# liuQuan98/EYOC

Measured on AMD Instinct MI355X. Metric: registered pairs/sec (30k-voxel KITTI pairs), higher is better.
Workload: dtype f32 (split16 products: fp32 storage/accumulation, 3 fp16 MFMAs on hi/lo-split operands per product); 1 GPU; 64 synthetic 30 cm KITTI-shaped pairs per step per GPU (mean 29894 voxels/cloud, ResUNetBN2C random-init, 5000-point NN, RANSAC 4000000 hypotheses/pair, planted inlier ratio 0.3, spconv math split16); parallelism=pairs sharded over 1 GPU(s), steps_in_flight=2

## Files before the change

eyoc_amd/_lib.py:

```python
from __future__ import annotations

import ctypes as C
import os
import threading

_HERE = os.path.dirname(os.path.abspath(__file__))
LIB_PATH = os.environ.get("EYOC_HIP_LIB") or os.path.join(_HERE, "lib", "libeyoc_hip.so")

MAX_LEVELS = 4
MAP_S1, MAP_DOWN, MAP_UP = 0, 1, 2


class MapsInfo(C.Structure):
    _fields_ = [("n_levels", C.c_int32), ("rows", C.c_int32 * MAX_LEVELS),
                ("pairs_s1", C.c_int64 * MAX_LEVELS), ("pairs_down", C.c_int64 * MAX_LEVELS),
                ("pairs_up", C.c_int64 * MAX_LEVELS), ("pairs_conv1", C.c_int64)]


class ModelDesc(C.Structure):
    _fields_ = [("in_channels", C.c_int32), ("out_channels", C.c_int32), ("conv1_kernel_size", C.c_int32),
                ("normalize_feature", C.c_int32), ("channels", C.c_int32 * 5), ("tr_channels", C.c_int32 * 5),
                ("bn_eps", C.c_float), ("expanded", C.c_int32)]


# ... 101 lines not shown
    "eyoc_spconv_grad_weight": (_i, [_vp, _vp, _i, _i, _vp, _i, _i, _vp, _i, _i, _vp, _vp, _sz, _vp]),
    "eyoc_spconv_pack_weights_split16": (_i, [_vp, _vp, _i, _i, _i, _vp, _vp]),
    "eyoc_spconv_ex": (_i, [_vp, _vp, _i, _i, _i, _vp, _i, _i, _vp, _i, _vp, _vp, _i, _i, _vp, _i, _i, _i, _vp, _vp]),
    "eyoc_spconv_select_split16_kernel": (_i, [_vp, _i]),
    "eyoc_spconv_select_st_kernel": (_i, [_vp, _i]),
    "eyoc_spconv_st_split_below": (_i, [_vp, _i]),
    "eyoc_spconv_st_group_rows": (_i, [_vp, _i]),
    "eyoc_spconv_st_ksplit": (_i, [_vp, _i]),
    "eyoc_spconv_local_rulebook_bytes": (_sz, [_i]),
    "eyoc_spconv_build_local_rulebook": (_i, [_vp, _vp, _i, _i, _vp, _vp, _vp]),
    "eyoc_spconv_staged": (_i, [_vp, _vp, _vp, _i, _i, _vp, _i, _i, _vp, _i, _vp, _vp, _i, _i, _vp, _i, _i, _vp, _vp]),
    "eyoc_split16_encode": (_i, [_vp, _vp, _i, _i, _i, _vp, _i, _vp]),
    "eyoc_split16_decode": (_i, [_vp, _vp, _i, _i, _i, _vp, _i, _vp]),
    "eyoc_model_set_math": (_i, [_vp, _i]),
    "eyoc_model_last_math": (_i, [_vp]),
    "eyoc_model_range_check": (_i, [_vp, _vp, C.POINTER(C.c_float)]),
    "eyoc_model_range_snapshot": (_i, [_vp, _vp, _vp]),
    "eyoc_model_set_progress_event": (_i, [_vp, _i, _vp]),
    "eyoc_model_set_probe": (_i, [_vp, _i]),
    "eyoc_spconv": (_i, [_vp, _vp, _i, _i, _vp, _i, _i, _vp, _i, _vp, _vp, _i, _i, _vp, _i, _vp]),
    "eyoc_spconv_sum": (_i, [_vp, _vp, _i, _i, _vp, _i, _i, _vp, _i, _vp, _i, _vp]),
    "eyoc_model_blob_floats": (_sz, [C.POINTER(ModelDesc)]),
    "eyoc_model_pack_host": (_i, [C.POINTER(ModelDesc), C.POINTER(LayerParams), _i, _vp, _sz]),
    "eyoc_model_create": (_i, [_vp, C.POINTER(ModelDesc), C.POINTER(LayerParams), _i, _vp, _sz, C.POINTER(_vp)]),
    "eyoc_model_destroy": (_i, [_vp]),
    "eyoc_model_repack_workspace_bytes": (_sz, [_vp]),
    "eyoc_model_repack_device": (_i, [_vp, _vp, C.POINTER(LayerParams), _i, _vp, _sz, _vp]),
    "eyoc_model_fuse_tail": (_i, [_vp, _i]),
    "eyoc_model_workspace_bytes": (_sz, [_vp, _vp]),
    "eyoc_model_forward": (_i, [_vp, _vp, _vp, _vp, _vp, _vp, _sz, _vp]),
    "eyoc_model_workspace_bytes_rows": (_sz, [_vp, _vp, _i]),
    "eyoc_model_forward_rows": (_i, [_vp, _vp, _vp, _vp, _vp, _i, _vp, _vp, _sz, _vp]),
    "eyoc_model_sampled_tail": (_i, [_vp, _i]),
    "eyoc_model_num_layers": (_i, [_vp]),
    "eyoc_model_layer_work": (_i, [_vp, _vp, _vp, _vp, C.POINTER(C.c_char_p), C.POINTER(C.c_int64),
                                   C.POINTER(C.c_double), C.POINTER(C.c_double), C.POINTER(C.c_double)]),
    "eyoc_model_set_timing": (_i, [_vp, _i]),
    "eyoc_model_layer_ms": (_i, [_vp, C.POINTER(C.c_float)]),
    "eyoc_model_timing_slot": (_i, [_vp, _i]),
    "eyoc_bn_workspace_bytes": (_sz, [_i, _i]),
    "eyoc_bn_train_forward": (_i, [_vp, _vp, _i, _i, _i, _vp, _vp, C.c_float, _i, _vp, _i, _vp, _vp, _sz, _vp]),
    "eyoc_bn_train_forward_running": (_i, [_vp, _vp, _i, _i, _i, _vp, _vp, C.c_float, _i, _vp, _i, _vp, _vp, _vp, C.c_float, _vp, _sz, _vp]),
    "eyoc_bn_train_backward": (_i, [_vp, _vp, _i, _vp, _i, _vp, _i, _i, _i, _vp, _vp, C.c_float, _vp, _i, _vp, _vp, _vp, _sz, _vp]),
    "eyoc_maps_gather_window": (_i, [_vp, _vp, _i, _vp, _i, _vp, _vp]),
    "eyoc_maps_gather_window_internal": (_i, [_vp, _vp, _i, _vp, _i, _vp, _vp]),
    "eyoc_knn_prefilter": (_i, [_vp, _i]),
    "eyoc_spconv_select_up_kernel": (_i, [_vp, _i]),
    "eyoc_spconv_upc_min_rows": (_i, [_vp, _i]),
    "eyoc_spconv_upc_tile_rows": (_i, [_i, _i]),
    "eyoc_spconv_upc_bytes": (_sz, [_i]),
    "eyoc_spconv_upc_build": (_i, [_vp, _vp, _i, _vp, _vp, _vp]),
    "eyoc_spconv_upc": (_i, [_vp, _vp, _vp, _i, _i, _vp, _i, _i, _vp, _i, _vp, _i, _vp, _i, _i, _vp, _vp]),
    "eyoc_spconv_select_conv1_kernel": (_i, [_vp, _i]),
    "eyoc_knn1": (_i, [_vp, _vp, _vp, _i, C.POINTER(C.c_int32), C.POINTER(C.c_int32), _i, _i, _vp, _vp, _vp]),
    "eyoc_pdist": (_i, [_vp, _vp, _i, _vp, _i, _i, _i, _vp, _vp]),
    "eyoc_kabsch_batched": (_i, [_vp, _vp, _vp, _vp, _i, _i, _vp, _vp]),
    "eyoc_irls_quad": (_i, [_vp, _vp, _vp, _vp, _i, _i, _vp, _vp]),
    "eyoc_irls_quad_batched": (_i, [_vp, _vp, _vp, _vp, _vp, C.POINTER(C.c_int32), C.POINTER(C.c_int32), _i, _i, _vp, _vp]),
    "eyoc_valid_metrics_batched": (_i, [_vp, _vp, _vp, _vp, C.POINTER(C.c_int32), C.POINTER(C.c_int32), _vp, C.POINTER(C.c_int32), _i, _vp, _vp,
                                        C.c_double, C.c_double, _vp, _vp]),
    "eyoc_ransac": (_i, [_vp, _vp, _vp, _vp, _i, C.POINTER(RansacParams), _vp, _vp]),
    "eyoc_maps_select_orders": (_i, [_vp, _i, _i]),
    "eyoc_ransac_select_pruning": (_i, [_vp, _i]),
    "eyoc_registration_accept_degenerate": (_i, [_vp, _i]),
    "eyoc_ransac_transform_store": (_i, [_vp, _i]),
    "eyoc_ransac_workspace_bytes": (_sz, [_vp, _i, _i, _i, _sz]),
# ... 173 lines not shown
```

eyoc_amd/csrc/common.h:

```cpp
#pragma once
#include <hip/hip_runtime.h>

#include <cstdarg>
#include <cstdint>
#include <cstdio>
#include <cstring>
#include <string>
#include <vector>

#include "../../include/eyoc_hip.h"

namespace eyoc {

void set_error(const char* fmt, ...);

#define EYOC_CHECK_HIP(expr)                                                               \
  do {                                                                                     \
    hipError_t _e = (expr);                                                                \
    if (_e != hipSuccess) {                                                                \
      eyoc::set_error("%s failed: %s (%s:%d)", #expr, hipGetErrorString(_e), __FILE__,    \
                      __LINE__);                                                           \
      return EYOC_ERR_HIP;                                                                 \
    }                                                                                      \
  } while (0)
// ... 25 lines not shown
}

struct eyoc_ctx {
  int device = 0;
  void* scratch = nullptr;
  size_t scratch_bytes = 0;
  void* pinned = nullptr;
  size_t pinned_bytes = 0;
  int ensure_scratch(size_t bytes, hipStream_t st);
  hipStream_t scratch_owner = nullptr;
  bool scratch_owned = false;
  hipEvent_t scratch_ev = nullptr;
  static constexpr int POOL = 8;
  hipStream_t pool[POOL] = {};
  hipEvent_t pool_done[POOL] = {};
  hipEvent_t pool_fork = nullptr;
  bool pool_ready = false;
  int ensure_pool();
  bool ransac_attr_set = false, sc2_attr_set = false;
  bool up_attr_set[2] = {false, false};
  int zorder_kbits = 17, zorder_bbits = 10;
  int sc2_list_cap = 1024, sc2_dense_x = 0;
  int sc2_legacy = 0;
  uint32_t fault_dup[32] = {}, fault_range[32] = {};
  struct Knobs {
    int maps_order_min_rows = 65536;
    int maps_window_shift = 18;
    int maps_s1_order = 1, maps_down_order = 0;
    int maps_internal_order = -1;
    int maps_lazy_tables = 1, maps_fused_levels = 1;
    int knn_prefilter = 1;
    int fuse_tail = 2;
    int sampled_tail = 1;
    int spconv_kernel = -1;
    int split16_kernel = 1;
    int up_kernel = 2;
    int s1_wide = 1;
    int st128_wide = 1;
    int down_kernel = 1;
    int upc_min_rows = 1 << 17;
    int conv1_kernel = 1;
    int st_group = 1;
    int st_variant = 1;
    int st_split_below = 1024;
    int st_cg_local = 1;
    int st_ksplit = 1;
    int ransac_store = 1 << 20;
    int ransac_prune = 2;
    int accept_degenerate = 0;
  } knobs;
};
inline const eyoc_ctx::Knobs& knobs_of(const eyoc_ctx* ctx) {
  static const eyoc_ctx::Knobs defaults;
  return ctx ? ctx->knobs : defaults;
}

namespace eyoc {

constexpr unsigned long long KEY_EMPTY = 0xFFFFFFFFFFFFFFFFull;
constexpr int COORD_BIAS = 1 << 17;
constexpr int VAL_UNSET = 0x7F7F7F7F;

struct HashTable {
  unsigned long long* keys;
  int* vals;
  unsigned int mask;
// ... 76 lines not shown
```

eyoc_amd/csrc/model.hip:

```cpp
#include <algorithm>
#include <cmath>
#include <cstdlib>

#include "spconv.h"

using namespace eyoc;

namespace {

enum MapSel { M_CONV1, M_S1, M_DOWN, M_UP, M_IDENT, M_AFFINE };

struct LayerPlan {
  std::string name;
  std::string norm;
  int K, cin, cout;
  MapSel map;
  int level;
  int out_level;
  int in_buf, in_col, out_buf, out_col, res_buf;
  int relu, l2norm, has_bias;
  size_t w_off = 0, b_off = 0;
  size_t w16_off = 0, s_off = 0;
};

enum Buf { B_IN = 0, B_X1, B_T1, B_CAT1, B_X2, B_T2, B_CAT2, B_X4, B_T4, B_CAT4, B_X8, B_T8, B_Y8, B_D4, B_DT4, B_D2,
           B_DT2, B_D1, B_DT1, B_H,
           B_U1, B_U2, B_U4, B_U8, B_UD4, B_UD2, B_UD1,
           B_OUT, B_COUNT };

struct BufPlan { int level, width; };

size_t pad64(size_t v) { return (v + 63) / 64 * 64; }

}

struct eyoc_model {
  eyoc_model_desc desc;
  std::vector<LayerPlan> layers;
  BufPlan bufs[B_COUNT];
  float* blob = nullptr;
  size_t blob_floats = 0;
  int math = -1;
  int last_math = 0;
  int timing = 0;
  std::vector<hipEvent_t> events;
  int slot = 0;
  int events_valid[2] = {0, 0};
  hipEvent_t progress_event = nullptr;
  int progress_layer = -1;
  unsigned int* range = nullptr;
  int probe = 0;
  int sampled_layer = -1, sampled_rows = 0;
};

namespace {

void build_plan(const eyoc_model_desc& d, std::vector<LayerPlan>& L, BufPlan* bufs) {
  const int* C = d.channels;
  const int* T = d.tr_channels;
  const int K1 = d.conv1_kernel_size * d.conv1_kernel_size * d.conv1_kernel_size;
  bufs[B_IN] = {0, d.in_channels};
  bufs[B_X1] = {0, C[1]}; bufs[B_T1] = {0, C[1]}; bufs[B_CAT1] = {0, T[2] + C[1]};
  bufs[B_X2] = {1, C[2]}; bufs[B_T2] = {1, C[2]}; bufs[B_CAT2] = {1, T[3] + C[2]};
  bufs[B_X4] = {2, C[3]}; bufs[B_T4] = {2, C[3]}; bufs[B_CAT4] = {2, T[4] + C[3]};
  bufs[B_X8] = {3, C[4]}; bufs[B_T8] = {3, C[4]}; bufs[B_Y8] = {3, C[4]};
  bufs[B_D4] = {2, T[4]}; bufs[B_DT4] = {2, T[4]};
  bufs[B_D2] = {1, T[3]}; bufs[B_DT2] = {1, T[3]};
  bufs[B_D1] = {0, T[2]}; bufs[B_DT1] = {0, T[2]};
  bufs[B_H] = {0, T[1]};
  bufs[B_OUT] = {0, d.out_channels};
  const int ex = d.expanded ? 1 : 0;
  bufs[B_U1] = {0, ex * C[1]}; bufs[B_U2] = {1, ex * C[2]}; bufs[B_U4] = {2, ex * C[3]}; bufs[B_U8] = {3, ex * C[4]};
  bufs[B_UD4] = {2, ex * T[4]}; bufs[B_UD2] = {1, ex * T[3]}; bufs[B_UD1] = {0, ex * T[2]};

  auto conv = [&](const char* name, const char* norm, int K, int cin, int cout, MapSel map, int level, int out_level,
                  int in_buf, int in_col, int out_buf, int out_col, int res_buf, int relu) {
    LayerPlan p;
    p.name = name; p.norm = norm; p.K = K; p.cin = cin; p.cout = cout; p.map = map; p.level = level;
    p.out_level = out_level; p.in_buf = in_buf; p.in_col = in_col; p.out_buf = out_buf; p.out_col = out_col;
    p.res_buf = res_buf; p.relu = relu; p.l2norm = 0; p.has_bias = 0;
    L.push_back(p);
  };
  auto block1 = [&](const std::string& name, int c, int level, int x_buf, int t_buf, int out_buf, int out_col) {
    conv((name + ".conv1").c_str(), (name + ".norm1").c_str(), 27, c, c, M_S1, level, level, x_buf, 0, t_buf, 0, -1, 1);
    conv((name + ".conv2").c_str(), (name + ".norm2").c_str(), 27, c, c, M_S1, level, level, t_buf, 0, out_buf, out_col,
// ... 543 lines not shown
      return KS_PART_BYTES;
  return 0;
}

size_t eyoc_model_workspace_bytes(const eyoc_model* m, const eyoc_maps* maps) {
  if (!m || !maps) return 0;
  size_t b = 0;
  for (int i = B_X1; i < B_OUT; ++i) b += align_up((size_t)maps->rows[m->bufs[i].level] * m->bufs[i].width * sizeof(float));
  b += align_up(ks_part_bytes(m, maps));
  return b + 256;
}

static size_t rows_region_floats(const eyoc_model* m, const eyoc_maps* maps, int n_rows) {
  return std::max((size_t)n_rows * 96, (size_t)maps->rows[0] * m->desc.out_channels);
}
static size_t rows_extra_floats(const eyoc_model* m, const eyoc_maps* maps, int n_rows) {
  const size_t need = rows_region_floats(m, maps, n_rows);
  return need <= (size_t)maps->rows[0] * m->bufs[B_X1].width ? 0 : need;
}

size_t eyoc_model_workspace_bytes_rows(const eyoc_model* m, const eyoc_maps* maps, int n_rows) {
  if (!m || !maps || n_rows < 0) return 0;
  return eyoc_model_workspace_bytes(m, maps) + align_up(rows_extra_floats(m, maps, n_rows) * sizeof(float)) +
         align_up(spconv_rows_scratch_bytes(maps->rows[0], n_rows));
}

int eyoc_model_sampled_tail(eyoc_ctx* ctx, int on) {
  if (!ctx) return -1;
  const int prev = ctx->knobs.sampled_tail;
  if (on == 0 || on == 1) ctx->knobs.sampled_tail = on;
  return prev;
}

int eyoc_model_num_layers(const eyoc_model* m) { return m ? (int)m->layers.size() : 0; }

int eyoc_model_set_math(eyoc_model* m, int mode) {
  EYOC_REQUIRE(m && mode >= -1 && mode <= 1, EYOC_ERR_INVALID, "eyoc_model_set_math: mode %d not in {-1, 0, 1}", mode);
  const int prev = m->math;
  m->math = mode;
  return prev + 1 ? prev + 2 : 1;
}

int eyoc_model_last_math(const eyoc_model* m) { return m ? m->last_math : -1; }

int eyoc_model_set_timing(eyoc_model* m, int on) {
  EYOC_REQUIRE(m, EYOC_ERR_INVALID, "eyoc_model_set_timing: NULL model");
  m->timing = on ? 1 : 0;
  m->events_valid[0] = m->events_valid[1] = 0;
  if (on && m->events.empty()) {
    m->events.resize(2 * (m->layers.size() + 1));
    for (auto& e : m->events) EYOC_CHECK_HIP(hipEventCreate(&e));
  }
  return EYOC_OK;
}

int eyoc_model_timing_slot(eyoc_model* m, int slot) {
  EYOC_REQUIRE(m && (slot == 0 || slot == 1), EYOC_ERR_INVALID, "eyoc_model_timing_slot: slot %d", slot);
  m->slot = slot;
  return EYOC_OK;
}

int eyoc_model_layer_ms(eyoc_model* m, float* ms) {
  EYOC_REQUIRE(m && ms, EYOC_ERR_INVALID, "eyoc_model_layer_ms: NULL argument");
  EYOC_REQUIRE(m->timing && m->events_valid[m->slot], EYOC_ERR_INVALID, "eyoc_model_layer_ms: no timed forward recorded in slot %d", m->slot);
  const hipEvent_t* ev = m->events.data() + (size_t)m->slot * (m->layers.size() + 1);
  EYOC_CHECK_HIP(hipEventSynchronize(ev[m->layers.size()]));
  for (size_t i = 0; i < m->layers.size(); ++i) EYOC_CHECK_HIP(hipEventElapsedTime(&ms[i], ev[i], ev[i + 1]));
  return EYOC_OK;
}

}

static int forward_impl(eyoc_ctx* ctx, const eyoc_model* mc, const eyoc_maps* maps, const float* feats_dev, float* out_dev, void* ws,
                        size_t ws_bytes, void* stream, const int64_t* rows_dev, int n_rows) {
  eyoc_model* m = const_cast<eyoc_model*>(mc);
  hipStream_t st = (hipStream_t)stream;
  float* buf[B_COUNT];
  Carver cv(ws, ws_bytes);
  buf[B_IN] = const_cast<float*>(feats_dev);
  buf[B_OUT] = out_dev;
  for (int i = B_X1; i < B_OUT; ++i) buf[i] = cv.take<float>((size_t)maps->rows[m->bufs[i].level] * m->bufs[i].width);
  const size_t ks_bytes = ks_part_bytes(m, maps);
  float* ks_part = ks_bytes ? cv.take<float>(ks_bytes / 4) : nullptr;
  float* rows_region = nullptr;
  void* rows_scratch = nullptr;
  if (rows_dev) {
    const size_t extra = rows_extra_floats(m, maps, n_rows);
    rows_region = extra ? cv.take<float>(extra) : buf[B_X1];
    rows_scratch = cv.take<unsigned char>(spconv_rows_scratch_bytes(maps->rows[0], n_rows));
    buf[B_OUT] = rows_region;
  }
  m->sampled_layer = -1;
  m->sampled_rows = 0;
  const int want = m->math;
  const bool split_ok = ctx->knobs.spconv_kernel != 0 && !(m->desc.normalize_feature && m->desc.out_channels > 64) &&
                        m->desc.channels[1] % 32 == 0;
  const bool split = split_ok && (want == 1 || (want < 0 && maps->rows[0] >= 8192));
  EYOC_REQUIRE(want != 1 || split, EYOC_ERR_INVALID,
               "eyoc_model_forward: split16 arithmetic is not available for this model / kernel selection");
  m->last_math = split ? 1 : 0;
  EYOC_CHECK_HIP(hipMemsetAsync(m->range, 0, 4, st));
  EYOC_CHECK_HIP(hipMemsetAsync(m->range + 4, 0, 8, st));
  hipEvent_t* ev = m->timing ? m->events.data() + (size_t)m->slot * (m->layers.size() + 1) : nullptr;
  if (m->timing) EYOC_CHECK_HIP(hipEventRecord(ev[0], st));
  bool progress_recorded = m->progress_event == nullptr;
  for (size_t li = 0; li < m->layers.size(); ++li) {
    const LayerPlan& p = m->layers[li];
    const int n_out = maps->rows[p.out_level];
    int rc;
    if (!progress_recorded && (int)li >= m->progress_layer) {
      EYOC_CHECK_HIP(hipEventRecord(m->progress_event, st));
      progress_recorded = true;
    }
    if (p.map == M_AFFINE) {
      rc = launch_affine(buf[p.in_buf] + p.in_col, m->bufs[p.in_buf].width, n_out, p.cout, m->blob + p.w_off, m->blob + p.b_off,
                         buf[p.out_buf] + p.out_col, m->bufs[p.out_buf].width, split, split ? m->range : nullptr, st);
    } else if (p.map == M_CONV1) {
      Conv1Args a;
      a.coords = maps->coords[0]; a.n = n_out; a.table = maps->table[0]; a.ks = m->desc.conv1_kernel_size;
      a.in = buf[p.in_buf]; a.cin = p.cin; a.w = m->blob + p.w_off; a.bias = m->blob + p.b_off; a.cout = p.cout;
      a.out = buf[p.out_buf] + p.out_col; a.ld_out = m->bufs[p.out_buf].width;
      a.out_split = split ? 1 : 0;
      a.ctx = ctx;
      a.range = split ? m->range : nullptr;
      a.wscale = m->blob + p.s_off;
      a.in_perm = maps->row_perm;
// ... 38 lines not shown
      a.n_in = maps->rows[m->bufs[p.in_buf].level];
      a.in = buf[p.in_buf] + p.in_col; a.ld_in = m->bufs[p.in_buf].width; a.cin = p.cin;
      a.w = m->blob + p.w_off; a.cout = p.cout; a.bias = m->blob + p.b_off;
      a.res = p.res_buf >= 0 ? buf[p.res_buf] : nullptr; a.ld_res = p.res_buf >= 0 ? m->bufs[p.res_buf].width : 0;
      a.relu = p.relu; a.l2norm = p.l2norm;
      a.out = buf[p.out_buf] + p.out_col; a.ld_out = m->bufs[p.out_buf].width;
      a.ctx = ctx;
      if (split) {
        a.math = 1;
        a.w = m->blob + p.w16_off;
        a.out_scale = m->blob + p.s_off;
        a.out_split = p.out_buf != B_OUT;
        a.range = m->range;
        if (p.map == M_S1 && p.cin >= 32 && p.cin % 32 == 0) { a.local = maps->local_s1[p.level]; a.ks_part = ks_part; }
        if (p.map == M_S1 && p.cin % 32 == 0 && p.cout % 128 == 0 && ctx->knobs.s1_wide) a.local128 = maps->local_s1w[p.level];
        if (p.map == M_DOWN && p.cin % 32 == 0 && p.cout % 64 == 0) a.local_down = maps->local_down[p.level];
        if (p.map == M_UP && p.cin % 32 == 0 && p.cout % 64 == 0) a.local_up = maps->local_up[p.level];
        if (p.map == M_UP && p.cin % 32 == 0 && p.cout % 64 == 0) a.local_upc = maps->local_upc[p.level];
      }
      if (p.out_buf == B_OUT) a.out_perm = maps->row_perm;
      if ((p.map == M_S1 || p.map == M_UP) && spconv_record_path(a) == 0)
        if ((rc = maps_ensure_table(const_cast<eyoc_maps*>(maps), p.map == M_S1 ? EYOC_MAP_S1 : EYOC_MAP_UP, p.level, st))) return rc;
      a.perm = p.map == M_UP ? maps->perm_up[p.level] : p.map == M_S1 ? maps->perm_s1[p.level]
               : p.map == M_DOWN ? maps->perm_down[p.level] : nullptr;
      if (split && ctx->knobs.fuse_tail == 2 && li + 3 == m->layers.size() && p.map == M_S1 && p.cout == 64) {
        const LayerPlan &q1 = m->layers[li + 1], &q2 = m->layers[li + 2];
        if (q1.map == M_IDENT && q1.K == 1 && q1.res_buf < 0 && q2.map == M_IDENT && q2.K == 1 && q2.in_buf == q1.out_buf && q2.res_buf < 0 &&
            !q2.relu && q2.out_buf == B_OUT && q1.out_col == 0 && tail_fusable(q1.cin, q1.cout, q2.cout) && q1.in_buf == p.out_buf &&
            q1.in_col == p.out_col && q1.cin == p.cout + 32 && spconv_record_path(a) == 1 &&
            (spconv_st_can_fuse_tail(a) || (rows_dev && ctx->knobs.sampled_tail))) {
          if (rows_dev && ctx->knobs.sampled_tail && maps->row_perm && spconv_rows_supported(a)) {
            EYOC_CHECK_HIP(hipMemsetAsync(m->range + 6, 0, 4, st));
            rc = launch_spconv_rows(a, a.local, maps->row_perm, rows_dev, n_rows, buf[q1.in_buf] + q1.in_col + p.cout,
                                    m->bufs[q1.in_buf].width, rows_region, rows_scratch, m->range + 6, st);
            if (!rc)
              rc = launch_tail_fused(rows_region, 96, n_rows, m->blob + q1.w16_off, m->blob + q1.s_off, m->blob + q1.b_off, q1.relu,
                                     m->blob + q2.w16_off, m->blob + q2.s_off, m->blob + q2.b_off, q2.l2norm, out_dev,
                                     m->desc.out_channels, nullptr, m->range, st);
            if (rc) return rc;
            m->sampled_layer = (int)li;
            m->sampled_rows = n_rows;
            if (m->timing)
              for (int e = 1; e <= 3; ++e) EYOC_CHECK_HIP(hipEventRecord(ev[li + e], st));
            li += 2;
            continue;
          }
          if (!spconv_st_can_fuse_tail(a)) goto unfused;
          a.tail.skip = buf[q1.in_buf] + q1.in_col + p.cout; a.tail.ld_skip = m->bufs[q1.in_buf].width;
          a.tail.w1 = m->blob + q1.w16_off; a.tail.s1 = m->blob + q1.s_off; a.tail.b1 = m->blob + q1.b_off; a.tail.relu1 = q1.relu;
          a.tail.w2 = m->blob + q2.w16_off; a.tail.s2 = m->blob + q2.s_off; a.tail.b2 = m->blob + q2.b_off; a.tail.l2norm = q2.l2norm;
          a.tail.out = buf[q2.out_buf] + q2.out_col; a.tail.ld_out = m->bufs[q2.out_buf].width; a.tail.out_perm = maps->row_perm;
          rc = launch_spconv(a, st);
          if (rc) return rc;
          if (m->timing)
            for (int e = 1; e <= 3; ++e) EYOC_CHECK_HIP(hipEventRecord(ev[li + e], st));
          li += 2;
          continue;
        }
      }
    unfused:
      rc = launch_spconv(a, st);
    }
    if (rc) return rc;
    if (m->timing) EYOC_CHECK_HIP(hipEventRecord(ev[li + 1], st));
  }
  if (!progress_recorded) EYOC_CHECK_HIP(hipEventRecord(m->progress_event, st));
  if (rows_dev && m->sampled_layer < 0)
// ... 85 lines not shown
```

eyoc_amd/csrc/spconv.h:

```cpp
#pragma once
#include "common.h"

namespace eyoc {

inline int spconv_ct(int cout) { return cout >= 128 ? 128 : cout; }
inline int spconv_cc(int cin, int ) { return cin % 64 == 0 ? 64 : 32; }

struct TailFuse {
  const float* skip = nullptr;
  int ld_skip = 0;
  const float *w1 = nullptr, *s1 = nullptr, *b1 = nullptr, *w2 = nullptr, *s2 = nullptr, *b2 = nullptr;
  int relu1 = 0, l2norm = 0;
  float* out = nullptr;
  int ld_out = 0;
  const int32_t* out_perm = nullptr;
};

struct SpconvArgs {
  const int32_t* nbr;
  int K, n_out;
  int n_in = 0;
  const float* in;
  int ld_in, cin;
  const float* w;
// ... 92 lines not shown
size_t local_rulebook_up_bytes(int n_out);
bool spconv_st_can_fuse_tail(const SpconvArgs& a);
int spconv_record_path(const SpconvArgs& a);
int build_local_rulebook_up(const int32_t* nbr_dev, int K, int n_out, unsigned char* out_dev, int* overflow_dev, hipStream_t st);
size_t upc_kept_bytes(int n_out);
size_t upc_scratch_bytes(int n_out);
int build_upc(const int32_t* nbr_dev, const int32_t* coords_dev, int stride, int n_out, unsigned char* ws, unsigned char* scratch, hipStream_t st, bool compact = false);
const int* upc_overflow_ptr(const unsigned char* ws);
int upc_set_tile_rows(int odd_axes, int rows);
int launch_spconv_upc(const SpconvArgs& a, const unsigned char* ws, hipStream_t st);
int st_variants();
size_t local_rulebook_bytes(int n_out);
int build_local_rulebook(const int32_t* nbr_dev, int K, int n_out, unsigned char* out_dev, int* overflow_dev, hipStream_t st, int group = 1);
struct DeriveSrc {
  const int32_t* coords = nullptr;
  const int32_t* parent = nullptr;
  const int32_t* children = nullptr;
  const int32_t* s1c = nullptr;
  int nc = 0, sh = 0;
  int32_t* up8 = nullptr;
};
size_t local_rulebook128_bytes(int n_out);
int build_local_rulebook128(const int32_t* nbr_dev, int K, int n_out, unsigned char* out_dev, int* overflow_dev, hipStream_t st, int group = 1);
int launch_spconv_st128(const SpconvArgs& a, const unsigned char* local_dev, hipStream_t st);
int build_local_rulebook_derived(const DeriveSrc& src, int n_out, unsigned char* out_dev, int* overflow_dev, hipStream_t st, int group = 1);
int launch_spconv_rs(const SpconvArgs& a, hipStream_t st);
bool tail_fusable(int cin1, int cmid, int cout);
int launch_tail_fused(const float* in, int ld_in, int n, const float* w1, const float* s1, const float* b1, int relu1, const float* w2,
                      const float* s2, const float* b2, int l2norm, float* out, int ld_out, const int32_t* out_perm, unsigned int* range,
                      hipStream_t st);
bool spconv_rows_supported(const SpconvArgs& a);
size_t spconv_rows_scratch_bytes(int n_level_rows, int n_rows);
int launch_spconv_rows(const SpconvArgs& a, const unsigned char* local_dev, const int32_t* row_perm, const int64_t* rows_dev, int n_rows,
                       const float* skip, int ld_skip, float* out, void* scratch, unsigned int* pairs, hipStream_t st);
int launch_take_rows(const float* in, int n, int c, const int64_t* rows_dev, int n_rows, float* out, hipStream_t st);
bool spconv_rs_fits(const SpconvArgs& a);
int launch_spconv_wave(const SpconvArgs& a, hipStream_t st);

struct Conv1Args {
  const int32_t* coords;
  int n;
  HashTable table;
  int ks;
  const float* in;
  int cin;
  const float* w;
  const float* bias;
  int cout;
  const float* wscale = nullptr;
  float* out;
  int ld_out;
  int out_split = 0;
  unsigned int* range = nullptr;
  const int32_t* in_perm = nullptr;
  const int32_t* parent;
  const int32_t* children;
  const int32_t* s1c;
  int nc;
  const unsigned char* local1 = nullptr;
  const eyoc_ctx* ctx = nullptr;
};
constexpr int ST_TILE = 256, ST_UMAX = 639, ST_UCAP = 1280, ST_NPASS = 2, ST_LOC_OFF = 16 + ST_UCAP * 4, ST_INV_OFF = 33152, ST_LR_BYTES = 33408;
int launch_conv1(const Conv1Args& a, hipStream_t st);
bool conv1_walks_octree(const Conv1Args& a);

}
```

eyoc_amd/csrc/spconv_rows.hip:

```cpp
#include "spconv.h"

using namespace eyoc;

namespace {

typedef float f32x4 __attribute__((ext_vector_type(4)));

constexpr int RW = 4;
constexpr int PASS_BIT = 28;

struct RowsArgs {
  SpconvArgs a;
  const unsigned char* local;
  const int32_t* rows;
  int n_rows;
  const float* skip;
  int ld_skip;
  float* out;
  const float* zero;
  unsigned int* pairs;
};

__global__ __launch_bounds__(RW * 64, 2) void spconv_rows_kernel(RowsArgs ra) {
  const SpconvArgs& a = ra.a;
  __shared__ __attribute__((aligned(16))) int nb[RW][27][64];
  const int lane = threadIdx.x & 63, wave = threadIdx.x >> 6;
  const int g = lane >> 4, j = lane & 15;
  const int base = ((int)blockIdx.x * RW + wave) * 64;
  if (base >= ra.n_rows) return;

  const int mine = base + lane;
  const int r = mine < ra.n_rows ? ra.rows[mine] : -1;
  int cnt = 0;
  bool second = false;
  {
    const unsigned char* lr = ra.local + (size_t)(r >= 0 ? r >> 8 : 0) * ST_LR_BYTES;
    const int n_u = reinterpret_cast<const int*>(lr)[0];
    const int* U = reinterpret_cast<const int*>(lr + 16);
    const unsigned short* loc = reinterpret_cast<const unsigned short*>(lr + ST_LOC_OFF);
    const int sl = lr[ST_INV_OFF + (r >= 0 ? r & 255 : 0)];
    const int ew = (sl >> 6) * 16 + (sl & 15), ec = (sl >> 4) & 3;
    const bool two = n_u > ST_UMAX;
    int e0[27], e1[27];
#pragma unroll
    for (int k = 0; k < 27; ++k) {
      e0[k] = loc[(k * 64 + ew) * 4 + ec] >> 6;
      e1[k] = two ? loc[((27 + k) * 64 + ew) * 4 + ec] >> 6 : ST_UMAX;
    }
#pragma unroll
    for (int k = 0; k < 27; ++k) {
      int v = -1;
      if (r >= 0 && n_u >= 0) {
        if (e0[k] < ST_UMAX) v = U[e0[k]];
        else if (e1[k] < ST_UMAX) v = U[ST_UMAX + e1[k]] | (1 << PASS_BIT);
      }
      nb[wave][k][4 * j + g] = v;
      cnt += v >= 0;
      second |= v >= (1 << PASS_BIT);
    }
  }
  const int n_pass = __ballot(second) != 0ull ? 2 : 1;
#pragma unroll
  for (int d = 32; d >= 1; d >>= 1) cnt += __shfl_xor(cnt, d, 64);
  if (lane == 0 && ra.pairs) atomicAdd(ra.pairs, (unsigned)cnt);
  __builtin_amdgcn_s_waitcnt(0xc07f);
  __builtin_amdgcn_wave_barrier();

  const int CC = a.cin % 64 == 0 ? 64 : 32 , JQ = CC / 16, ncc = a.cin / CC, tile4 = CC * 64 / 4;
  const int nqb = a.cin / 32, n_steps = nqb * 27;
  const char* wb = reinterpret_cast<const char*>(a.w) + lane * 16;
  const char* inb = reinterpret_cast<const char*>(a.in) + g * 16;
  const char* zb = reinterpret_cast<const char*>(ra.zero) + g * 16;
  const size_t row_bytes = (size_t)a.ld_in * 4;

  f32x4 acc[4][4];
#pragma unroll
  for (int c = 0; c < 4; ++c)
#pragma unroll
    for (int t = 0; t < 4; ++t) acc[c][t] = f32x4{0.f, 0.f, 0.f, 0.f};

  auto load = [&](int pass, int s, half8_t (&X)[4][2], half8_t (&W)[4][2]) -> bool {
    const int qb = s / 27, k = s - qb * 27;
    const int4 nv = *reinterpret_cast<const int4*>(&nb[wave][k][4 * j]);
    const int v[4] = {nv.x, nv.y, nv.z, nv.w};
    bool any = false;
#pragma unroll
    for (int c = 0; c < 4; ++c) {
      const bool has = v[c] >= 0 && (v[c] >> PASS_BIT) == pass;
      any |= has;
      const char* p = has ? inb + (size_t)(v[c] & ((1 << PASS_BIT) - 1)) * row_bytes + qb * 128 : zb;
      X[c][0] = *reinterpret_cast<const half8_t*>(p);
      X[c][1] = *reinterpret_cast<const half8_t*>(p + SPLIT16_LO);
    }
    const int cc = (qb * 32) / CC, qp = ((qb * 32) % CC) / 32;
    const char* wp = wb + ((size_t)((k * ncc + cc) * tile4) + 2 * qp * 64) * 16;
#pragma unroll
    for (int t = 0; t < 4; ++t)
#pragma unroll
      for (int p = 0; p < 2; ++p) W[t][p] = *reinterpret_cast<const half8_t*>(wp + (t * JQ + p) * 1024);
    return __ballot(any) != 0ull;
  };
  auto multiply = [&](const half8_t (&X)[4][2], const half8_t (&W)[4][2]) {
#pragma unroll
    for (int term = 0; term < 3; ++term)
#pragma unroll
      for (int c = 0; c < 4; ++c)
#pragma unroll
        for (int t = 0; t < 4; ++t)
          acc[c][t] = __builtin_amdgcn_mfma_f32_16x16x32_f16(W[t][term == 2 ? 1 : 0], X[c][term == 1 ? 1 : 0], acc[c][t], 0, 0, 0);
  };

  half8_t XA[4][2], XB[4][2], WA[4][2], WB[4][2];
  for (int pass = 0; pass < n_pass; ++pass) {
    bool anyA = load(pass, 0, XA, WA), anyB = false;
    for (int s = 0; s < n_steps; s += 2) {
      if (s + 1 < n_steps) anyB = load(pass, s + 1, XB, WB);
      if (anyA) multiply(XA, WA);
      if (s + 1 >= n_steps) break;
      if (s + 2 < n_steps) anyA = load(pass, s + 2, XA, WA);
      if (anyB) multiply(XB, WB);
    }
  }

  const float os = a.out_scale ? *a.out_scale : 1.0f;
  float4 b4[4];
#pragma unroll
  for (int t = 0; t < 4; ++t) b4[t] = a.bias ? *reinterpret_cast<const float4*>(a.bias + 16 * t + 4 * g) : make_float4(0.f, 0.f, 0.f, 0.f);
  float mx = 0.f;
#pragma unroll
  for (int c = 0; c < 4; ++c) {
    const int i = base + 16 * c + j;
    if (i >= ra.n_rows) continue;
    const int o = ra.rows[i];
    float* dst = ra.out + (size_t)i * (a.cout + 32);
#pragma unroll
    for (int t = 0; t < 4; ++t) {
      const int ch = 16 * t + 4 * g;
      float4 v = make_float4(acc[c][t][0] * os + b4[t].x, acc[c][t][1] * os + b4[t].y, acc[c][t][2] * os + b4[t].z,
                             acc[c][t][3] * os + b4[t].w);
      if (a.res) {
        const float4 q = split16_load4(a.res + (size_t)o * a.ld_res, ch);
        v.x += q.x; v.y += q.y; v.z += q.z; v.w += q.w;
      }
      if (a.relu) { v.x = fmaxf(v.x, 0.f); v.y = fmaxf(v.y, 0.f); v.z = fmaxf(v.z, 0.f); v.w = fmaxf(v.w, 0.f); }
      split16_track(mx, v);
      split16_store4(dst, ch, v);
    }
    const uint4* sp = reinterpret_cast<const uint4*>(ra.skip + (size_t)o * ra.ld_skip);
    uint4* dp = reinterpret_cast<uint4*>(dst + a.cout);
    dp[g] = sp[g];
    dp[4 + g] = sp[4 + g];
  }
  split16_report(a.range, mx);
}

__global__ __launch_bounds__(256) void k_invert_perm(const int32_t* __restrict__ perm, int n, int32_t* __restrict__ inv) {
  const int i = blockIdx.x * 256 + threadIdx.x;
  if (i < n) inv[perm[i]] = i;
}

__global__ __launch_bounds__(256) void k_rows_internal(const long long* __restrict__ rows, int n_rows, const int32_t* __restrict__ inv, int n,
                                                       int32_t* __restrict__ out, float* __restrict__ zero) {
  const int i = blockIdx.x * 256 + threadIdx.x;
  if (blockIdx.x == 0 && threadIdx.x < 64) zero[threadIdx.x] = 0.f;
  if (i >= n_rows) return;
  long long r = rows[i];
  r = r < 0 ? 0 : r >= n ? n - 1 : r;
  out[i] = inv ? inv[r] : (int32_t)r;
}

__global__ __launch_bounds__(256) void k_take_rows(const float* __restrict__ in, int n, int c4, const long long* __restrict__ rows, int n_rows,
                                                   float* __restrict__ out) {
  const long long t = (long long)blockIdx.x * 256 + threadIdx.x;
  const long long i = t / c4;
  const int q = (int)(t % c4);
  if (i >= n_rows) return;
  long long r = rows[i];
  r = r < 0 ? 0 : r >= n ? n - 1 : r;
  reinterpret_cast<float4*>(out)[i * c4 + q] = reinterpret_cast<const float4*>(in)[r * c4 + q];
}

}

namespace eyoc {

bool spconv_rows_supported(const SpconvArgs& a) {
  return a.math == 1 && a.K == 27 && a.cout == 64 && a.cin % 32 == 0 && a.ld_in % 32 == 0 && a.out_split && !a.l2norm && !a.out_perm &&
         a.n_in < (1 << 24) && (!a.res || a.ld_res % 32 == 0);
}

size_t spconv_rows_scratch_bytes(int n_level_rows, int n_rows) {
  return align_up((size_t)n_level_rows * 4) + align_up((size_t)n_rows * 4) + 256;
}

int launch_spconv_rows(const SpconvArgs& a, const unsigned char* local_dev, const int32_t* row_perm, const int64_t* rows_dev, int n_rows,
                       const float* skip, int ld_skip, float* out, void* scratch, unsigned int* pairs, hipStream_t st) {
  EYOC_REQUIRE(spconv_rows_supported(a) && local_dev && rows_dev && skip && out && scratch && ld_skip % 32 == 0, EYOC_ERR_INVALID,
               "spconv_rows: unsupported layer");
  if (n_rows <= 0) return EYOC_OK;
  Carver cv(scratch, spconv_rows_scratch_bytes(a.n_out, n_rows));
  int32_t* inv = cv.take<int32_t>((size_t)a.n_out);
  int32_t* internal = cv.take<int32_t>((size_t)n_rows);
  float* zero = cv.take<float>(64);
  if (row_perm) hipLaunchKernelGGL(k_invert_perm, dim3(cdiv(a.n_out, 256)), dim3(256), 0, st, row_perm, a.n_out, inv);
  hipLaunchKernelGGL(k_rows_internal, dim3(cdiv(n_rows, 256)), dim3(256), 0, st, (const long long*)rows_dev, n_rows,
                     row_perm ? inv : (const int32_t*)nullptr, a.n_out, internal, zero);
  RowsArgs ra{a, local_dev, internal, n_rows, skip, ld_skip, out, zero, pairs};
  hipLaunchKernelGGL(spconv_rows_kernel, dim3(cdiv(n_rows, RW * 64)), dim3(RW * 64), 0, st, ra);
  EYOC_CHECK_HIP(hipGetLastError());
  return EYOC_OK;
}

int launch_take_rows(const float* in, int n, int c, const int64_t* rows_dev, int n_rows, float* out, hipStream_t st) {
  EYOC_REQUIRE(in && rows_dev && out && c % 4 == 0 && n > 0, EYOC_ERR_INVALID, "take_rows: bad argument");
  if (n_rows <= 0) return EYOC_OK;
  hipLaunchKernelGGL(k_take_rows, dim3(cdiv((long long)n_rows * (c / 4), 256)), dim3(256), 0, st, in, n, c / 4, (const long long*)rows_dev,
                     n_rows, out);
  EYOC_CHECK_HIP(hipGetLastError());
  return EYOC_OK;
}

}
```

include/eyoc_hip.h:

```cpp
#ifndef EYOC_HIP_H
#define EYOC_HIP_H

#include <stddef.h>
#include <stdint.h>

#ifdef __cplusplus
extern "C" {
#endif

typedef struct eyoc_ctx eyoc_ctx;
typedef struct eyoc_maps eyoc_maps;
typedef struct eyoc_model eyoc_model;

typedef enum {
  EYOC_OK = 0,
  EYOC_ERR_INVALID = -1,
  EYOC_ERR_HIP = -2,
  EYOC_ERR_WORKSPACE = -3,
  EYOC_ERR_DUPLICATE = -4,
  EYOC_ERR_RANGE = -5
} eyoc_status;

#define EYOC_MAX_LEVELS 4
#define EYOC_VERSION 111
// ... 113 lines not shown
  int32_t expanded;
} eyoc_model_desc;

typedef struct {
  const char* name;
  const float* kernel;
  int32_t K, cin, cout;
  const float* bias;
  const float* bn_weight;
  const float* bn_bias;
  const float* bn_mean;
  const float* bn_var;
} eyoc_layer_params;

size_t eyoc_model_blob_floats(const eyoc_model_desc* desc);
int eyoc_model_pack_host(const eyoc_model_desc* desc, const eyoc_layer_params* layers, int n_layers,
                         float* blob_host, size_t blob_floats);
int eyoc_model_create(eyoc_ctx* ctx, const eyoc_model_desc* desc, const eyoc_layer_params* layers,
                      int n_layers, float* blob_dev, size_t blob_floats, eyoc_model** out);
int eyoc_model_destroy(eyoc_model* model);
size_t eyoc_model_repack_workspace_bytes(const eyoc_model* model);
int eyoc_model_repack_device(eyoc_ctx* ctx, eyoc_model* model, const eyoc_layer_params* layers, int n_layers,
                             void* workspace_dev, size_t workspace_bytes, void* stream);
int eyoc_model_fuse_tail(eyoc_ctx* ctx, int on);
size_t eyoc_model_workspace_bytes(const eyoc_model* model, const eyoc_maps* maps);
int eyoc_model_forward(eyoc_ctx* ctx, const eyoc_model* model, const eyoc_maps* maps,
                       const float* feats_dev, float* out_dev, void* workspace_dev,
                       size_t workspace_bytes, void* stream);
size_t eyoc_model_workspace_bytes_rows(const eyoc_model* model, const eyoc_maps* maps, int n_rows);
int eyoc_model_forward_rows(eyoc_ctx* ctx, const eyoc_model* model, const eyoc_maps* maps, const float* feats_dev,
                            const int64_t* rows_dev, int n_rows, float* out_dev, void* workspace_dev, size_t workspace_bytes,
                            void* stream);
int eyoc_model_sampled_tail(eyoc_ctx* ctx, int on);
int eyoc_model_num_layers(const eyoc_model* model);
int eyoc_model_layer_work(eyoc_ctx* ctx, const eyoc_model* model, const eyoc_maps* maps, void* stream,
                          const char** names, int64_t* pairs, double* flops, double* gather_bytes,
                          double* compulsory_bytes);
int eyoc_model_set_math(eyoc_model* model, int mode);
int eyoc_model_last_math(const eyoc_model* model);
int eyoc_model_range_check(eyoc_model* model, void* stream, float* max_abs);
int eyoc_model_range_snapshot(eyoc_model* model, uint32_t* words_host, void* stream);
int eyoc_model_set_progress_event(eyoc_model* model, int layer, void* hip_event);
int eyoc_model_set_probe(eyoc_model* model, int on);
int eyoc_model_set_timing(eyoc_model* model, int on);
int eyoc_model_layer_ms(eyoc_model* model, float* ms );
int eyoc_model_timing_slot(eyoc_model* model, int slot);

int eyoc_knn_prefilter(eyoc_ctx* ctx, int mode);
int eyoc_knn1(eyoc_ctx* ctx, const float* A_dev, const float* B_dev, int c, const int32_t* seg_a,
              const int32_t* seg_b, int nseg, int dist_type, int64_t* idx_dev, float* dist_dev,
              void* stream);

int eyoc_gather_rows(eyoc_ctx* ctx, const float* F_dev, int ld, int c, const int64_t* sel_dev, int n,
                     const float* G_dev, float beta, float* out_dev, void* stream);

int eyoc_dotmax(eyoc_ctx* ctx, const float* A_dev, const float* B_dev, int c, const int32_t* seg_a,
                const int32_t* seg_b, int nseg, int64_t* idx_dev, float* weight_dev, void* stream);

int eyoc_knn2(eyoc_ctx* ctx, const float* A_dev, const float* B_dev, int c, const int32_t* seg_a,
              const int32_t* seg_b, int nseg, int64_t* idx_dev, float* d1_dev, float* d2_dev, void* stream);

int eyoc_lowe_topk(eyoc_ctx* ctx, const float* d1_dev, const float* d2_dev, int n, int k, int64_t* idx_out_dev,
                   float* w_out_dev, void* stream);
int eyoc_pair_filter(eyoc_ctx* ctx, int mode, const float* P0_dev, const float* P1_dev, const int64_t* idx0_dev,
                     const int64_t* idx1_dev, int m, const float* T_dev, float radius, int64_t* pairs_out_dev,
                     int32_t* n_out_dev, void* stream);
// ... 168 lines not shown
```

Measured before the change: 3385 pairs/s.

## Restructure sampled-rows spconv to skip empty offsets and stage gathers via LDS

The sampled-rows sparse conv kernel now builds per-wave bitmasks of which kernel offsets have any neighbor in each pass and iterates only over those offsets, instead of all 27 per channel block. Neighbor inputs are gathered as 8 contiguous 16-byte chunks per lane and transposed through a swizzled LDS buffer into the MFMA operand layout, which replaces the earlier scattered 4x2 loads. An optional sort of sampled rows by internal index (rows_order knob, off by default) is added to improve gather locality, at the cost of extra scratch and a radix sort. The skipping and staging apply by default; the extra LDS traffic and wave barriers per step may cost something.

Measured after the change: 3406 pairs/s, median of 6. No clear change (+0.6%).

```diff
diff --git a/eyoc_amd/_lib.py b/eyoc_amd/_lib.py
--- a/eyoc_amd/_lib.py
+++ b/eyoc_amd/_lib.py
@@ -157,6 +157,8 @@
     "eyoc_model_workspace_bytes_rows": (_sz, [_vp, _vp, _i]),
     "eyoc_model_forward_rows": (_i, [_vp, _vp, _vp, _vp, _vp, _i, _vp, _vp, _sz, _vp]),
     "eyoc_model_sampled_tail": (_i, [_vp, _i]),
+    "eyoc_model_rows_order": (_i, [_vp, _i]),
+    "eyoc_model_last_rows_sorts": (_i, [_vp]),
     "eyoc_model_num_layers": (_i, [_vp]),
     "eyoc_model_layer_work": (_i, [_vp, _vp, _vp, _vp, C.POINTER(C.c_char_p), C.POINTER(C.c_int64),
                                    C.POINTER(C.c_double), C.POINTER(C.c_double), C.POINTER(C.c_double)]),
diff --git a/eyoc_amd/csrc/common.h b/eyoc_amd/csrc/common.h
--- a/eyoc_amd/csrc/common.h
+++ b/eyoc_amd/csrc/common.h
@@ -81,6 +81,7 @@
     int knn_prefilter = 1;
     int fuse_tail = 2;
     int sampled_tail = 1;
+    int rows_order = 0;
     int spconv_kernel = -1;
     int split16_kernel = 1;
     int up_kernel = 2;
diff --git a/eyoc_amd/csrc/model.hip b/eyoc_amd/csrc/model.hip
--- a/eyoc_amd/csrc/model.hip
+++ b/eyoc_amd/csrc/model.hip
@@ -51,6 +51,7 @@
   unsigned int* range = nullptr;
   int probe = 0;
   int sampled_layer = -1, sampled_rows = 0;
+  int sampled_sorts = 0;
 };
 
 namespace {
@@ -660,6 +661,15 @@
   return prev;
 }
 
+int eyoc_model_rows_order(eyoc_ctx* ctx, int mode) {
+  if (!ctx) return -1;
+  const int prev = ctx->knobs.rows_order;
+  if (mode >= 0 && mode <= 2) ctx->knobs.rows_order = mode;
+  return prev;
+}
+
+int eyoc_model_last_rows_sorts(const eyoc_model* m) { return m ? m->sampled_sorts : -1; }
+
 int eyoc_model_num_layers(const eyoc_model* m) { return m ? (int)m->layers.size() : 0; }
 
 int eyoc_model_set_math(eyoc_model* m, int mode) {
@@ -720,6 +730,7 @@
   }
   m->sampled_layer = -1;
   m->sampled_rows = 0;
+  m->sampled_sorts = 0;
   const int want = m->math;
   const bool split_ok = ctx->knobs.spconv_kernel != 0 && !(m->desc.normalize_feature && m->desc.out_channels > 64) &&
                         m->desc.channels[1] % 32 == 0;
@@ -824,7 +835,7 @@
           if (rows_dev && ctx->knobs.sampled_tail && maps->row_perm && spconv_rows_supported(a)) {
             EYOC_CHECK_HIP(hipMemsetAsync(m->range + 6, 0, 4, st));
             rc = launch_spconv_rows(a, a.local, maps->row_perm, rows_dev, n_rows, buf[q1.in_buf] + q1.in_col + p.cout,
-                                    m->bufs[q1.in_buf].width, rows_region, rows_scratch, m->range + 6, st);
+                                    m->bufs[q1.in_buf].width, rows_region, rows_scratch, m->range + 6, &m->sampled_sorts, st);
             if (!rc)
               rc = launch_tail_fused(rows_region, 96, n_rows, m->blob + q1.w16_off, m->blob + q1.s_off, m->blob + q1.b_off, q1.relu,
                                      m->blob + q2.w16_off, m->blob + q2.s_off, m->blob + q2.b_off, q2.l2norm, out_dev,
diff --git a/eyoc_amd/csrc/spconv.h b/eyoc_amd/csrc/spconv.h
--- a/eyoc_amd/csrc/spconv.h
+++ b/eyoc_amd/csrc/spconv.h
@@ -148,7 +148,7 @@
 bool spconv_rows_supported(const SpconvArgs& a);
 size_t spconv_rows_scratch_bytes(int n_level_rows, int n_rows);
 int launch_spconv_rows(const SpconvArgs& a, const unsigned char* local_dev, const int32_t* row_perm, const int64_t* rows_dev, int n_rows,
-                       const float* skip, int ld_skip, float* out, void* scratch, unsigned int* pairs, hipStream_t st);
+                       const float* skip, int ld_skip, float* out, void* scratch, unsigned int* pairs, int* n_sorts, hipStream_t st);
 int launch_take_rows(const float* in, int n, int c, const int64_t* rows_dev, int n_rows, float* out, hipStream_t st);
 bool spconv_rs_fits(const SpconvArgs& a);
 int launch_spconv_wave(const SpconvArgs& a, hipStream_t st);
diff --git a/eyoc_amd/csrc/spconv_rows.hip b/eyoc_amd/csrc/spconv_rows.hip
--- a/eyoc_amd/csrc/spconv_rows.hip
+++ b/eyoc_amd/csrc/spconv_rows.hip
@@ -1,3 +1,5 @@
+#include <algorithm>
+
 #include "spconv.h"
 
 using namespace eyoc;
@@ -13,6 +15,7 @@
   SpconvArgs a;
   const unsigned char* local;
   const int32_t* rows;
+  const int32_t* order;
   int n_rows;
   const float* skip;
   int ld_skip;
@@ -24,15 +27,17 @@
 __global__ __launch_bounds__(RW * 64, 2) void spconv_rows_kernel(RowsArgs ra) {
   const SpconvArgs& a = ra.a;
   __shared__ __attribute__((aligned(16))) int nb[RW][27][64];
+  __shared__ __attribute__((aligned(16))) half8_t xs[RW][64][8];
   const int lane = threadIdx.x & 63, wave = threadIdx.x >> 6;
   const int g = lane >> 4, j = lane & 15;
+  const int r3 = lane >> 3, pc = lane & 7;
   const int base = ((int)blockIdx.x * RW + wave) * 64;
   if (base >= ra.n_rows) return;
 
   const int mine = base + lane;
-  const int r = mine < ra.n_rows ? ra.rows[mine] : -1;
+  const int r = mine < ra.n_rows ? ra.rows[ra.order ? ra.order[mine] : mine] : -1;
   int cnt = 0;
-  bool second = false;
+  unsigned int mine0 = 0u, mine1 = 0u;
   {
     const unsigned char* lr = ra.local + (size_t)(r >= 0 ? r >> 8 : 0) * ST_LR_BYTES;
     const int n_u = reinterpret_cast<const int*>(lr)[0];
@@ -54,23 +59,28 @@
         if (e0[k] < ST_UMAX) v = U[e0[k]];
         else if (e1[k] < ST_UMAX) v = U[ST_UMAX + e1[k]] | (1 << PASS_BIT);
       }
-      nb[wave][k][4 * j + g] = v;
+      nb[wave][k][8 * (lane & 7) + (lane >> 3)] = v;
       cnt += v >= 0;
-      second |= v >= (1 << PASS_BIT);
-    }
-  }
-  const int n_pass = __ballot(second) != 0ull ? 2 : 1;
-#pragma unroll
-  for (int d = 32; d >= 1; d >>= 1) cnt += __shfl_xor(cnt, d, 64);
+      mine0 |= (unsigned)(v >= 0 && v < (1 << PASS_BIT)) << k;
+      mine1 |= (unsigned)(v >= (1 << PASS_BIT)) << k;
+    }
+  }
+#pragma unroll
+  for (int d = 32; d >= 1; d >>= 1) {
+    cnt += __shfl_xor(cnt, d, 64);
+    mine0 |= __shfl_xor(mine0, d, 64);
+    mine1 |= __shfl_xor(mine1, d, 64);
+  }
+  const unsigned int steps[2] = {(unsigned)__builtin_amdgcn_readfirstlane((int)mine0), (unsigned)__builtin_amdgcn_readfirstlane((int)mine1)};
   if (lane == 0 && ra.pairs) atomicAdd(ra.pairs, (unsigned)cnt);
   __builtin_amdgcn_s_waitcnt(0xc07f);
   __builtin_amdgcn_wave_barrier();
 
   const int CC = a.cin % 64 == 0 ? 64 : 32 , JQ = CC / 16, ncc = a.cin / CC, tile4 = CC * 64 / 4;
-  const int nqb = a.cin / 32, n_steps = nqb * 27;
+  const int nqb = a.cin / 32;
   const char* wb = reinterpret_cast<const char*>(a.w) + lane * 16;
-  const char* inb = reinterpret_cast<const char*>(a.in) + g * 16;
-  const char* zb = reinterpret_cast<const char*>(ra.zero) + g * 16;
+  const char* inb = reinterpret_cast<const char*>(a.in) + pc * 16;
+  const char* zb = reinterpret_cast<const char*>(ra.zero) + pc * 16;
   const size_t row_bytes = (size_t)a.ld_in * 4;
 
   f32x4 acc[4][4];
@@ -79,18 +89,14 @@
 #pragma unroll
     for (int t = 0; t < 4; ++t) acc[c][t] = f32x4{0.f, 0.f, 0.f, 0.f};
 
-  auto load = [&](int pass, int s, half8_t (&X)[4][2], half8_t (&W)[4][2]) -> bool {
-    const int qb = s / 27, k = s - qb * 27;
-    const int4 nv = *reinterpret_cast<const int4*>(&nb[wave][k][4 * j]);
-    const int v[4] = {nv.x, nv.y, nv.z, nv.w};
-    bool any = false;
-#pragma unroll
-    for (int c = 0; c < 4; ++c) {
-      const bool has = v[c] >= 0 && (v[c] >> PASS_BIT) == pass;
-      any |= has;
-      const char* p = has ? inb + (size_t)(v[c] & ((1 << PASS_BIT) - 1)) * row_bytes + qb * 128 : zb;
-      X[c][0] = *reinterpret_cast<const half8_t*>(p);
-      X[c][1] = *reinterpret_cast<const half8_t*>(p + SPLIT16_LO);
+  auto load = [&](int pass, int qb, int k, half8_t (&S)[8], half8_t (&W)[4][2]) {
+    const int4 n0 = *reinterpret_cast<const int4*>(&nb[wave][k][8 * r3]), n1 = *reinterpret_cast<const int4*>(&nb[wave][k][8 * r3 + 4]);
+    const int v[8] = {n0.x, n0.y, n0.z, n0.w, n1.x, n1.y, n1.z, n1.w};
+#pragma unroll
+    for (int t = 0; t < 8; ++t) {
+      const bool has = v[t] >= 0 && (v[t] >> PASS_BIT) == pass;
+      const char* p = has ? inb + (size_t)(v[t] & ((1 << PASS_BIT) - 1)) * row_bytes + qb * 128 : zb;
+      S[t] = *reinterpret_cast<const half8_t*>(p);
     }
     const int cc = (qb * 32) / CC, qp = ((qb * 32) % CC) / 32;
     const char* wp = wb + ((size_t)((k * ncc + cc) * tile4) + 2 * qp * 64) * 16;
@@ -98,7 +104,18 @@
     for (int t = 0; t < 4; ++t)
 #pragma unroll
       for (int p = 0; p < 2; ++p) W[t][p] = *reinterpret_cast<const half8_t*>(wp + (t * JQ + p) * 1024);
-    return __ballot(any) != 0ull;
+  };
+  auto stage = [&](const half8_t (&S)[8], half8_t (&X)[4][2]) {
+#pragma unroll
+    for (int t = 0; t < 8; ++t) xs[wave][8 * t + r3][pc ^ r3] = S[t];
+    __builtin_amdgcn_fence(__ATOMIC_RELEASE, "wavefront");
+    __builtin_amdgcn_wave_barrier();
+#pragma unroll
+    for (int c = 0; c < 4; ++c)
+#pragma unroll
+      for (int h = 0; h < 2; ++h) X[c][h] = xs[wave][16 * c + j][(4 * h + g) ^ (j & 7)];
+    __builtin_amdgcn_fence(__ATOMIC_ACQUIRE, "wavefront");
+    __builtin_amdgcn_wave_barrier();
   };
   auto multiply = [&](const half8_t (&X)[4][2], const half8_t (&W)[4][2]) {
 #pragma unroll
@@ -110,15 +127,28 @@
           acc[c][t] = __builtin_amdgcn_mfma_f32_16x16x32_f16(W[t][term == 2 ? 1 : 0], X[c][term == 1 ? 1 : 0], acc[c][t], 0, 0, 0);
   };
 
-  half8_t XA[4][2], XB[4][2], WA[4][2], WB[4][2];
-  for (int pass = 0; pass < n_pass; ++pass) {
-    bool anyA = load(pass, 0, XA, WA), anyB = false;
+  half8_t S[8], X[4][2], WA[4][2], WB[4][2];
+  for (int pass = 0; pass < 2; ++pass) {
+    const unsigned int mask = steps[pass];
+    if (!mask) continue;
+    const int n_steps = nqb * __builtin_popcount(mask);
+    int qb = 0;
+    unsigned int rem = mask;
+    auto next = [&](half8_t (&W)[4][2]) {
+      if (!rem) { ++qb; rem = mask; }
+      const int k = __builtin_ctz(rem);
+      rem &= rem - 1;
+      load(pass, qb, k, S, W);
+    };
+    next(WA);
     for (int s = 0; s < n_steps; s += 2) {
-      if (s + 1 < n_steps) anyB = load(pass, s + 1, XB, WB);
-      if (anyA) multiply(XA, WA);
+      stage(S, X);
+      if (s + 1 < n_steps) next(WB);
+      multiply(X, WA);
       if (s + 1 >= n_steps) break;
-      if (s + 2 < n_steps) anyA = load(pass, s + 2, XA, WA);
-      if (anyB) multiply(XB, WB);
+      stage(S, X);
+      if (s + 2 < n_steps) next(WA);
+      multiply(X, WB);
     }
   }
 
@@ -129,8 +159,9 @@
   float mx = 0.f;
 #pragma unroll
   for (int c = 0; c < 4; ++c) {
-    const int i = base + 16 * c + j;
-    if (i >= ra.n_rows) continue;
+    const int e = base + 16 * c + j;
+    if (e >= ra.n_rows) continue;
+    const int i = ra.order ? ra.order[e] : e;
     const int o = ra.rows[i];
     float* dst = ra.out + (size_t)i * (a.cout + 32);
 #pragma unroll
@@ -160,13 +191,19 @@
 }
 
 __global__ __launch_bounds__(256) void k_rows_internal(const long long* __restrict__ rows, int n_rows, const int32_t* __restrict__ inv, int n,
-                                                       int32_t* __restrict__ out, float* __restrict__ zero) {
+                                                       int32_t* __restrict__ out, float* __restrict__ zero, unsigned int* __restrict__ key,
+                                                       int key_shift, int32_t* __restrict__ val) {
   const int i = blockIdx.x * 256 + threadIdx.x;
   if (blockIdx.x == 0 && threadIdx.x < 64) zero[threadIdx.x] = 0.f;
   if (i >= n_rows) return;
   long long r = rows[i];
   r = r < 0 ? 0 : r >= n ? n - 1 : r;
-  out[i] = inv ? inv[r] : (int32_t)r;
+  const int32_t o = inv ? inv[r] : (int32_t)r;
+  out[i] = o;
+  if (key) {
+    key[i] = (unsigned int)o >> key_shift;
+    val[i] = i;
+  }
 }
 
 __global__ __launch_bounds__(256) void k_take_rows(const float* __restrict__ in, int n, int c4, const long long* __restrict__ rows, int n_rows,
@@ -189,23 +226,48 @@
          a.n_in < (1 << 24) && (!a.res || a.ld_res % 32 == 0);
 }
 
+static int rows_key_bits(int n_level_rows, int key_shift) {
+  int bits = 1;
+  while (bits < 31 && ((long long)1 << bits) < (long long)n_level_rows) ++bits;
+  return std::max(bits - key_shift, 1);
+}
+static size_t rows_sort_tmp_bytes(int n_level_rows, int n_rows) {
+  return std::max(sort_rows_tmp_bytes(n_rows, rows_key_bits(n_level_rows, 0)), sort_rows_tmp_bytes(n_rows, rows_key_bits(n_level_rows, 8)));
+}
+
 size_t spconv_rows_scratch_bytes(int n_level_rows, int n_rows) {
-  return align_up((size_t)n_level_rows * 4) + align_up((size_t)n_rows * 4) + 256;
+  return align_up((size_t)n_level_rows * 4) + align_up((size_t)n_rows * 4) + 256 + 4 * align_up((size_t)n_rows * 4) +
+         align_up(rows_sort_tmp_bytes(n_level_rows, n_rows));
 }
 
 int launch_spconv_rows(const SpconvArgs& a, const unsigned char* local_dev, const int32_t* row_perm, const int64_t* rows_dev, int n_rows,
-                       const float* skip, int ld_skip, float* out, void* scratch, unsigned int* pairs, hipStream_t st) {
+                       const float* skip, int ld_skip, float* out, void* scratch, unsigned int* pairs, int* n_sorts, hipStream_t st) {
   EYOC_REQUIRE(spconv_rows_supported(a) && local_dev && rows_dev && skip && out && scratch && ld_skip % 32 == 0, EYOC_ERR_INVALID,
                "spconv_rows: unsupported layer");
+  if (n_sorts) *n_sorts = 0;
   if (n_rows <= 0) return EYOC_OK;
+  const int order_mode = knobs_of(a.ctx).rows_order;
+  const int key_shift = order_mode == 2 ? 8 : 0;
   Carver cv(scratch, spconv_rows_scratch_bytes(a.n_out, n_rows));
   int32_t* inv = cv.take<int32_t>((size_t)a.n_out);
   int32_t* internal = cv.take<int32_t>((size_t)n_rows);
   float* zero = cv.take<float>(64);
+  unsigned int* key_in = cv.take<unsigned int>((size_t)n_rows);
+  unsigned int* key_out = cv.take<unsigned int>((size_t)n_rows);
+  int32_t* val_in = cv.take<int32_t>((size_t)n_rows);
+  int32_t* order = cv.take<int32_t>((size_t)n_rows);
+  const size_t tmp_bytes = rows_sort_tmp_bytes(a.n_out, n_rows);
+  void* tmp = cv.take<unsigned char>(tmp_bytes);
+  EYOC_REQUIRE(cv.ok(), EYOC_ERR_WORKSPACE, "spconv_rows: scratch too small");
   if (row_perm) hipLaunchKernelGGL(k_invert_perm, dim3(cdiv(a.n_out, 256)), dim3(256), 0, st, row_perm, a.n_out, inv);
   hipLaunchKernelGGL(k_rows_internal, dim3(cdiv(n_rows, 256)), dim3(256), 0, st, (const long long*)rows_dev, n_rows,
-                     row_perm ? inv : (const int32_t*)nullptr, a.n_out, internal, zero);
-  RowsArgs ra{a, local_dev, internal, n_rows, skip, ld_skip, out, zero, pairs};
+                     row_perm ? inv : (const int32_t*)nullptr, a.n_out, internal, zero, order_mode ? key_in : (unsigned int*)nullptr, key_shift,
+                     val_in);
+  if (order_mode) {
+    if (int rc = sort_rows_by_key(tmp, tmp_bytes, key_in, key_out, val_in, order, n_rows, rows_key_bits(a.n_out, key_shift), st)) return rc;
+    if (n_sorts) *n_sorts = 1;
+  }
+  RowsArgs ra{a, local_dev, internal, order_mode ? order : (const int32_t*)nullptr, n_rows, skip, ld_skip, out, zero, pairs};
   hipLaunchKernelGGL(spconv_rows_kernel, dim3(cdiv(n_rows, RW * 64)), dim3(RW * 64), 0, st, ra);
   EYOC_CHECK_HIP(hipGetLastError());
   return EYOC_OK;
diff --git a/include/eyoc_hip.h b/include/eyoc_hip.h
--- a/include/eyoc_hip.h
+++ b/include/eyoc_hip.h
@@ -169,6 +169,8 @@
                             const int64_t* rows_dev, int n_rows, float* out_dev, void* workspace_dev, size_t workspace_bytes,
                             void* stream);
 int eyoc_model_sampled_tail(eyoc_ctx* ctx, int on);
+int eyoc_model_rows_order(eyoc_ctx* ctx, int mode);
+int eyoc_model_last_rows_sorts(const eyoc_model* model);
 int eyoc_model_num_layers(const eyoc_model* model);
 int eyoc_model_layer_work(eyoc_ctx* ctx, const eyoc_model* model, const eyoc_maps* maps, void* stream,
                           const char** names, int64_t* pairs, double* flops, double* gather_bytes,
```
